# dmn-sjk/cones_perception

Hardware: NVIDIA B200
Metric: points/sec at 130k-pt scans (frames/sec and p50 frame latency in extra keys) (higher is better)
Workload: dtype f32

## Files before the change

### cones_perception_b200/csrc/frame_kernels.cuh

```cuda
#pragma once
#include "cluster_kernels.cuh"
#include "common.cuh"
#include "stream_kernels.cuh"
#include "voxel_kernels.cuh"

namespace cp {

constexpr int kFrameThreadsMax = 512;

#ifdef CP_PHASE_CLOCKS
#define CP_PHASE(name)                                                          \
  do {                                                                          \
    __syncthreads();                                                            \
    if (tid == 0 && f == 0 && clk_n < 16) {                                     \
      clk_name[clk_n] = name;                                                   \
      clk_t[clk_n++] = clock64();                                               \
    }                                                                           \
  } while (0)
#else
#define CP_PHASE(name) do { } while (0)
#endif

struct FrameArgs {
  u32 n_frames;
  const uint8_t* in;
  Layout layout;
  Geom geom;
  const u32* mask;
  const u32* rowmax;
  const u32* low_key;
  CropK crop;
  GroundK gk;
  u32* rows_loaded;
  const u32* c_off;
  u32* gcount;
  int pad_survives;
  VoxelK vk;
  ClusterK ck;
  VoxelFrame* vf;
  u32* v_off;
  u32* k_off;
  u32* ncomp_f;
  u32* kcount_f;
  u32* ncrop_f;
  ClusterRec* slots;
  ClusterRec* direct_out;
  u32 direct_cap;
  u32* nvox_f;
  u32* fc;
  int counted_ground;
  u64* desc_v;
  Ctl* ctl;
  u32* ticket;
  float4* tap_vox;
  u32 tap_vox_cap;
  u32* tap_keys;
  u32* tap_order;
  i32* tap_labels;
};

template <int CMAX, int VMAX, int T>
struct FrameSmem {
// ... 70 lines not shown
    total += t;
  }
  return woff + inc - v;
}

template <int CMAX, int VMAX, int MODE, int T>
__device__ __forceinline__ void frame_process(const FrameArgs& a, FrameSmem<CMAX, VMAX, T>& s, const u32 f) {
  constexpr int kFrameThreads = T;
  const u32 tid = threadIdx.x;
  const int lane = lane_id(), warp = tid >> 5;
  {
#ifdef CP_PHASE_CLOCKS
    const char* clk_name[16];
    long long clk_t[16];
    int clk_n = 0;
    const long long clk_0 = clock64();
#endif
    u32 tile0, ntiles, npts;
    u64 first;
    if (a.geom.uniform_n) {
      tile0 = f * a.geom.tpf;
      ntiles = a.geom.tpf;
      npts = a.geom.uniform_n;
      first = (u64)f * a.geom.uniform_n;
    } else {
      tile0 = a.geom.frame_tile0[f];
      ntiles = (f + 1 < a.n_frames ? a.geom.frame_tile0[f + 1] : a.geom.n_tiles) - tile0;
      npts = a.geom.frame_n[f];
      first = a.geom.frame_off[f];
    }
    const u32 c0 = a.c_off ? a.c_off[f] : 0u;

    if (tid < 8) s.bbox[tid] = tid < 4 ? 0xFFFFFFFFu : 0u;
    if (tid == 0) {
      s.slow = 0;
      s.gkept = 0;
    }
    const bool fused = a.mask == nullptr;
    const bool do_ground = fused && a.gk.do_ground != 0;
    if (warp == 0) {
      float t = 0.0f;
      if (do_ground && lane < kNSect) {
        t = __double2float_ru((double)ord2f(__ldcg(&a.low_key[f * kSectStride + lane])) + 0.1);
        s.thr[lane] = t;
      }
      float mn = (do_ground && lane < kNSect) ? t : __int_as_float(0x7f800000);
      float mx = (do_ground && lane < kNSect) ? t : -__int_as_float(0x7f800000);
#pragma unroll
      for (int o2 = 16; o2; o2 >>= 1) {
        mn = fminf(mn, __shfl_xor_sync(kFull, mn, o2));
        mx = fmaxf(mx, __shfl_xor_sync(kFull, mx, o2));
      }
      if (lane == 0) {
        s.thr[31] = do_ground ? mn : -__int_as_float(0x7f800000);
        s.thr[30] = do_ground ? mx : -__int_as_float(0x7f800000);
      }
    }
    __syncthreads();
    u32 C = 0;
    {
      constexpr u32 CH = 4u * CMAX;
      constexpr u32 RPT = CH / kFrameThreads;
      static_assert(CH % kFrameThreads == 0 && RPT % 8 == 0 && RPT <= 32, "chunk rows per thread");
      static_assert(sizeof(s.u) >= CH * sizeof(unsigned short), "live-row list must fit the scratch union");
      u32* mword = reinterpret_cast<u32*>(&s.px[0]);
      unsigned short* liverow = reinterpret_cast<unsigned short*>(&s.u);
      const u32 nrows = (npts + 31u) >> 5;
      const float thr_min = s.thr[31], thr_max = s.thr[30];
      const u32 key_min = f2ord(thr_min);
      const bool skipping = do_ground && a.rowmax != nullptr;
      u32 mnx = 0xFFFFFFFFu, mny = 0xFFFFFFFFu, mnz = 0xFFFFFFFFu, mxx = 0, mxy = 0, mxz = 0;
      u32 gkept = 0;
      for (u32 cb = 0; cb < nrows; cb += CH) {
        const u32 nr = nrows - cb < CH ? nrows - cb : CH;
        const u32 r0 = tid * RPT;
        u32 w[RPT];
        if (!fused) {
#pragma unroll
          for (u32 q = 0; q < RPT; q += 4) {
            uint4 m = make_uint4(0u, 0u, 0u, 0u);
            if (r0 + q < nr) m = *reinterpret_cast<const uint4*>(a.mask + (u64)tile0 * kTileWords + cb + r0 + q);
            w[q] = m.x; w[q + 1] = m.y; w[q + 2] = m.z; w[q + 3] = m.w;
          }
        } else {
          u32 live = 0;
#pragma unroll
          for (u32 q = 0; q < RPT; q += 4) {
            uint4 m = make_uint4(0xFFFFFFFFu, 0xFFFFFFFFu, 0xFFFFFFFFu, 0xFFFFFFFFu);
            if (skipping && r0 + q < nr)
              m = __ldcg(reinterpret_cast<const uint4*>(a.rowmax + (u64)tile0 * kTileWords + cb + r0 + q));
            live |= (m.x >= key_min ? 1u : 0u) << q;
            live |= (m.y >= key_min ? 1u : 0u) << (q + 1);
            live |= (m.z >= key_min ? 1u : 0u) << (q + 2);
            live |= (m.w >= key_min ? 1u : 0u) << (q + 3);
          }
          if (r0 + RPT > nr) live &= r0 < nr ? (0xFFFFFFFFu >> (32u - (nr - r0))) : 0u;
#pragma unroll
          for (u32 q = 0; q < RPT; ++q) mword[r0 + q] = 0u;
          u32 nlive;
          u32 lp = block_excl_scan<T>(__popc(live), s.wsum, nlive);
          while (live) {
            const u32 b = (u32)__ffs(live) - 1u;
            live &= live - 1;
            liverow[lp++] = (unsigned short)(r0 + b);
          }
          if (tid == 0) s.nlive = nlive;
          __syncthreads();
          CP_PHASE("live rows");
          constexpr u32 KB = T == 256 ? 4 : 8;
          for (u32 e0 = (u32)warp * KB; e0 < nlive; e0 += (kFrameThreads / 32) * KB) {
            float4 p[KB];
            u32 row[KB];
#pragma unroll
            for (u32 j = 0; j < KB; ++j) {
              row[j] = e0 + j < nlive ? (u32)liverow[e0 + j] : 0xFFFFFFFFu;
              const u32 i = (cb + row[j]) * 32u + lane;
              p[j] = (row[j] != 0xFFFFFFFFu && i < npts) ? load_point<MODE>(a.in, first + i, a.layout)
                                                          : make_float4(0.f, 0.f, -__int_as_float(0x7f800000), 0.f);
            }
#pragma unroll
            for (u32 j = 0; j < KB; ++j) {
              if (row[j] == 0xFFFFFFFFu) break;
              const u32 i = (cb + row[j]) * 32u + lane;
              const u32 bal = __ballot_sync(kFull, keep_point(p[j], i < npts, a.crop, a.gk, s.thr, thr_min, thr_max, gkept));
              if (lane == 0) mword[row[j]] = bal;
            }
          }
          __syncthreads();
          CP_PHASE("pass 2");
// ... 515 lines not shown
```

### cones_perception_b200/csrc/pipeline.cu

```cuda
#include "../../include/conesgpu.h"

#include <math.h>
#include <stdio.h>
#include <string.h>
#include <time.h>

#include <algorithm>
#include <memory>
#include <new>
#include <string>
#include <vector>

#include "cluster_front.cuh"
#include "cluster_kernels.cuh"
#include "color_kernels.cuh"
#include "color_net.cuh"
#include "common.cuh"
#include "copy_pool.hpp"
#include "frame_kernels.cuh"
#include "plane_kernels.cuh"
#include "radix_sort.cuh"
#include "single_frame.cuh"
#include "stream_kernels.cuh"
#include "tflite_reader.hpp"
// ... 130 lines not shown
  const uint8_t* in_ptr = nullptr;
  Layout layout{};
  const uint8_t* run_in = nullptr;
  Layout run_layout{};
  bool plane_on = false;
  cp_plane_params plane{};
  double plane_cos = 0.0;
  bool plane_run = false;
  bool plane_valid = false;
  u32 plane_frames = 0, plane_h = 0;
  PlaneBufs pb{};
  HostGeom hg;
  u32 *d_frame_n = nullptr, *d_frame_tile0 = nullptr, *d_tile_frame = nullptr;
  u64* d_frame_off = nullptr;
  u32 *d_low_key = nullptr, *d_bbox = nullptr, *d_c_off = nullptr, *d_gcount = nullptr, *d_v_off = nullptr;
  u32 *d_ncomp_f = nullptr, *d_kcount_f = nullptr, *d_k_off = nullptr;
  VoxelFrame* d_vf = nullptr;
  float4* d_pts = nullptr;
  u32 *d_src = nullptr, *d_frame = nullptr;
  u64 *d_keys_a = nullptr, *d_keys_b = nullptr, *d_okeys_a = nullptr, *d_okeys_b = nullptr;
  u32 *d_vals_a = nullptr, *d_vals_b = nullptr, *d_ovals_a = nullptr, *d_ovals_b = nullptr;
  u32 *d_sort_hdr = nullptr, *d_sort_state = nullptr;
  u32 *d_vstart = nullptr, *d_cstart = nullptr, *d_comp_start = nullptr;
  float4* d_vox = nullptr;
  u32 *d_vox_frame = nullptr, *d_parent = nullptr, *d_label = nullptr;
  u64* d_hkeys = nullptr;
  u32* d_hvals = nullptr;
  ClusterRec* d_clusters = nullptr;
  u32 *d_mask = nullptr, *d_tile_count = nullptr, *d_tile_excl = nullptr;
  float* d_thr_f = nullptr;
  u32* d_rowmax = nullptr;
  bool rowmax_valid = false;
  bool use_rowskip = true;
  bool use_single = true;
  bool self_published = false;
  bool graph_self_published = false;
  u64 hint_c = 0, hint_v = 0;
  cp_ground_params rp_ground{};
  bool rp_has_ground = false;
  bool tail_priority = false;
  int prio_low = 0;
  int k1_ctas_per_sm = 0;
  int frame_ctas_per_sm = 0;
  bool tile_ctas = true;
  u32 run_sgrid = 0;
  int stream_ctas_per_sm = 8;
  u64 *d_desc_a = nullptr, *d_desc_b = nullptr, *d_desc_c = nullptr, *d_desc_d = nullptr;
  u32 *d_tap_keys = nullptr, *d_tap_order = nullptr;
  i32* d_tap_labels = nullptr;
  uint8_t* h_stage[2] = {nullptr, nullptr};
  bool stage_streaming = true;
  int stage_threads = 1;
  std::unique_ptr<CopyPool> copy_pool;
  Ctl* h_ctl = nullptr;
  u32* h_frame_u32 = nullptr;
  std::vector<void*> dev_allocs, pin_allocs;
};

namespace {

#define CK(call)                                                                              \
  do {                                                                                        \
    cudaError_t e_ = (call);                                                                  \
    if (e_ != cudaSuccess) {                                                                  \
      char buf_[512];                                                                         \
      snprintf(buf_, sizeof(buf_), "%s:%d %s -> %s", __FILE__, __LINE__, #call,               \
               cudaGetErrorString(e_));                                                       \
      h->err = buf_;                                                                          \
      return CP_E_CUDA;                                                                       \
    }                                                                                         \
  } while (0)

template <typename T>
cp_status dalloc(cp_handle* h, T** p, size_t count) {
  void* q = nullptr;
// ... 106 lines not shown
  k->r2 = (float)((double)tol_f * (double)tol_f);
  if (!(tol_f > 0.0f) || !isfinite(tol_f)) {
    h->err = "cone_width/cone_height give a non-positive or non-finite cluster tolerance";
    return CP_E_PARAM;
  }
  const double edge = (double)tol_f * 0.505;
  double reach = fabs(d->distance_treshold_max);
  if (!(reach < 1e6)) {
    h->err = "distance_treshold_max must be finite and below 1e6 m";
    return CP_E_PARAM;
  }
  reach += 4 * edge;
  const u64 nx = (u64)ceil(2.0 * reach / edge) + 2;
  k->inv_h = (float)(1.0 / ((double)tol_f * 1.01));
  k->inv_g = (float)(1.0 / edge);
  k->origin = (float)reach;
  k->nx = (u32)nx;
  const u64 cells = (u64)n_frames * nx * nx * nx;
  if (nx > (1u << 20) || ceil_log2_host(cells) > 60) {
    h->err = "neighbour grid too large for 64-bit cell keys";
    return CP_E_PARAM;
  }
  *csort_bits = ceil_log2_host(cells);
  if (*csort_bits == 0) *csort_bits = 1;
  k->min_size = d->min_cluster_size < 0 ? 0u : (u32)d->min_cluster_size;
  k->max_size = d->max_cluster_size < 0 ? 0u : (u32)d->max_cluster_size;
  k->frame_bits = ceil_log2_host(n_frames);
  k->size_bits = ceil_log2_host((u64)k->max_size + 1);
  *osort_bits = k->frame_bits + k->size_bits + 1;
  return CP_OK;
}

__global__ void init_kernel(Ctl* ctl, u32 n_frames, float default_low, u32* low_key, u32* bbox, u32* c_off,
                            u32* gcount, u32* ncomp_f, u32* kcount_f, u64* desc_a, u32 na, u64* desc_b,
                            u64* desc_c, u64* desc_d, u32 nb) {
  const u32 t = blockIdx.x * blockDim.x + threadIdx.x, stride = gridDim.x * blockDim.x;
  if (t == 0) {
    Ctl z;
    memset(&z, 0, sizeof(z));
    *ctl = z;
    c_off[0] = 0;
  }
  const u32 lk = f2ord(default_low);
  for (u32 i = t; i < n_frames * kSectStride; i += stride) low_key[i] = lk;
  for (u32 i = t; i < n_frames * 8; i += stride) bbox[i] = ((i & 7u) < 4u) ? 0xFFFFFFFFu : 0u;
  for (u32 i = t; i < n_frames; i += stride) {
    gcount[i] = 0;
    ncomp_f[i] = 0;
    kcount_f[i] = 0;
    c_off[i + 1] = 0;
  }
  for (u32 i = t; i < na; i += stride) desc_a[i] = 0;
  for (u32 i = t; i < nb; i += stride) {
    desc_b[i] = 0;
    desc_c[i] = 0;
    desc_d[i] = 0;
  }
}

__global__ void tap_voxel_kernel(const Ctl* ctl, const u64* keys_a, const u64* keys_b, const u32* vals_a,
                                 const u32* vals_b, u32* tap_keys, u32* tap_order) {
  const u32 n = ctl->n_surv;
  const bool inb = sorted_in_b(ctl->vsort_bits);
  const u64* keys = inb ? keys_b : keys_a;
  const u32* vals = inb ? vals_b : vals_a;
  const u64 mask = (ctl->voxel_key_bits >= 64) ? ~0ull : ((1ull << ctl->voxel_key_bits) - 1ull);
  for (u32 i = blockIdx.x * blockDim.x + threadIdx.x; i < n; i += gridDim.x * blockDim.x) {
    tap_keys[i] = (u32)(keys[i] & mask);
    tap_order[i] = vals[i];
  }
}

cp_status check_view(cp_handle* h, const cp_cloud_view* v) {
  if (!v) {
    h->err = "NULL cloud view";
    return CP_E_PARAM;
  }
  const u64 n = (u64)v->width * v->height;
  if (n && !v->data) {
    h->err = "cloud view has points but a NULL data pointer";
// ... 97 lines not shown
  g.frame_off = h->d_frame_off;
  g.tile_frame = h->d_tile_frame;
  g.frame_tile0 = h->d_frame_tile0;
  return g;
}

u64 hinted(u64 cap, u64 hint) { return hint ? std::min<u64>(cap, 2 * hint + 8192) : cap; }

u32 grid_for(u64 work, u32 block, int sms, int per_sm) {
  u64 b = (work + block - 1) / block;
  if (b == 0) b = 1;
  const u64 cap = (u64)sms * per_sm;
  return (u32)(b < cap ? b : cap);
}

void launch_keep_mask(cp_handle* h, const Geom& g, const CropK& c, const GroundK& gk, u32 grid) {
  MaskOut mo;
  mo.mask = h->d_mask;
  mo.tile_count = h->d_tile_count;
  mo.gcount = h->d_gcount;
  mo.rows_loaded = &h->d_ctl->rows_loaded;
  if (gk.do_ground) {
    ground_thresholds_kernel<<<(g.n_frames + 127) / 128, 128, 0, h->stream>>>(g.n_frames, h->d_low_key, h->d_thr_f);
    h->launches++;
  }
  cudaMemsetAsync(h->d_mask, 0, sizeof(u32) * (size_t)g.n_tiles * kTileWords, h->stream);
  cudaMemsetAsync(h->d_tile_count, 0, sizeof(u32) * g.n_tiles, h->stream);
  if (h->stage_timing) cudaEventRecord(h->ev_k[2], h->stream);
  const u32 total_warps = (u32)h->sms * 4u * kStreamWarps;
  u32 split_log2 = 0;
  while (split_log2 < 3 && (((u64)g.n_tiles * 2u) << (split_log2 + 1)) <= total_warps) ++split_log2;
  if (split_log2) grid = grid_for((((u64)g.n_tiles * 2u) << split_log2) * 32u, kStreamThreads, h->sms, h->stream_ctas_per_sm);
  const u32* rm = h->rowmax_valid ? h->d_rowmax : nullptr;
  switch (h->run_layout.mode) {
    case 0: keep_mask_kernel<0><<<grid, kStreamThreads, 0, h->stream>>>(h->run_in, h->run_layout, g, c, gk, h->d_thr_f, rm, mo, split_log2); break;
    case 1: keep_mask_kernel<1><<<grid, kStreamThreads, 0, h->stream>>>(h->run_in, h->run_layout, g, c, gk, h->d_thr_f, rm, mo, split_log2); break;
    default: keep_mask_kernel<2><<<grid, kStreamThreads, 0, h->stream>>>(h->run_in, h->run_layout, g, c, gk, h->d_thr_f, rm, mo, split_log2); break;
  }
  if (h->stage_timing) cudaEventRecord(h->ev_k[3], h->stream);
  h->launches++;
  h->masked = true;
}

void launch_scan_gather(cp_handle* h, const Geom& g, const GroundK& gk, u32 cap) {
  GatherOut go;
  go.pts = h->d_pts;
  go.src = h->d_src;
  go.frame = h->d_frame;
  go.cap = cap;
  go.bbox_key = h->d_bbox;
  go.out32 = nullptr;
  const u32 stiles = (g.n_tiles + kScanTile - 1) / kScanTile;
  tile_scan_kernel<<<(h->tile_ctas || stiles < (u32)h->sms * 4) ? stiles : (u32)h->sms * 4, kScanThreads, 0, h->stream>>>(
      g, h->d_tile_count, h->d_tile_excl, h->d_c_off, h->d_desc_a, h->d_ctl, cap);
  const u32 ggrid = grid_for((u64)g.n_tiles * 32, 256, h->sms, 8);
  switch (h->run_layout.mode) {
    case 0: gather_survivors_kernel<0><<<ggrid, 256, 0, h->stream>>>(h->run_in, h->run_layout, g, gk, h->d_mask, h->d_tile_count, h->d_tile_excl, go); break;
    case 1: gather_survivors_kernel<1><<<ggrid, 256, 0, h->stream>>>(h->run_in, h->run_layout, g, gk, h->d_mask, h->d_tile_count, h->d_tile_excl, go); break;
    default: gather_survivors_kernel<2><<<ggrid, 256, 0, h->stream>>>(h->run_in, h->run_layout, g, gk, h->d_mask, h->d_tile_count, h->d_tile_excl, go); break;
  }
  h->launches += 2;
  h->gathered = true;
}
template <bool OUT32>
void launch_mask_compact(cp_handle* h, const Geom& g, const CropK& c, const GroundK& gk, u32 cap, uint8_t* out32) {
  GatherOut go;
  go.pts = h->d_pts;
  go.src = h->d_src;
  go.frame = h->d_frame;
  go.cap = cap;
  go.bbox_key = h->d_bbox;
// ... 83 lines not shown
void launch_front_fused(cp_handle* h, const Geom& g, const CropK& c, const GroundK& gk) {
  MaskOut mo;
  mo.mask = h->d_mask;
  mo.tile_count = h->d_tile_count;
  mo.gcount = h->d_gcount;
  mo.rows_loaded = &h->d_ctl->rows_loaded;
  if (h->fused_grid == 0) {
    int occ = 0;
    cudaOccupancyMaxActiveBlocksPerMultiprocessor(&occ, front_fused_kernel<0>, kStreamThreads, 0);
    if (occ < 1) occ = 1;
    h->fused_grid = (u32)(h->sms * occ);
  }
  FusedArgs fa;
  const u32 gf = (h->fused_grid + g.tpf - 1) / g.tpf;
  fa.group_tiles = gf * g.tpf;
  fa.n_groups = (g.n_frames + gf - 1) / gf;
  fa.done = h->d_done;
  fa.ticket = h->d_frame_ticket + 1;
  cudaMemsetAsync(h->d_done, 0, sizeof(u32) * g.n_frames, h->stream);
  cudaMemsetAsync(h->d_frame_ticket + 1, 0, sizeof(u32), h->stream);
  const u32 items = fa.n_groups * fa.group_tiles * 2u;
  const u32 grid = items < h->fused_grid ? items : h->fused_grid;
  if (h->stage_timing) cudaEventRecord(h->ev_k[0], h->stream);
  switch (h->run_layout.mode) {
    case 0: front_fused_kernel<0><<<grid, kStreamThreads, 0, h->stream>>>(h->run_in, h->run_layout, g, c, gk, h->d_low_key, mo, fa); break;
    case 1: front_fused_kernel<1><<<grid, kStreamThreads, 0, h->stream>>>(h->run_in, h->run_layout, g, c, gk, h->d_low_key, mo, fa); break;
    default: front_fused_kernel<2><<<grid, kStreamThreads, 0, h->stream>>>(h->run_in, h->run_layout, g, c, gk, h->d_low_key, mo, fa); break;
  }
  if (h->stage_timing) cudaEventRecord(h->ev_k[1], h->stream);
  h->launches++;
}

template <int MODE>
void launch_sector_min_mode(cp_handle* h, const Geom& g, u32 grid) {
  if (!h->tail_priority) {
    ground_sector_min_kernel<MODE><<<grid, kStreamThreads, 0, h->stream>>>(h->run_in, h->run_layout, g, h->d_low_key, h->d_rowmax);
    return;
  }
  cudaLaunchConfig_t cfg = {};
  cfg.gridDim = dim3(grid);
  cfg.blockDim = dim3(kStreamThreads);
  cfg.stream = h->stream;
  cudaLaunchAttribute at[1];
  at[0].id = cudaLaunchAttributePriority;
  at[0].val.priority = h->prio_low;
  cfg.attrs = at;
  cfg.numAttrs = 1;
  cudaLaunchKernelEx(&cfg, ground_sector_min_kernel<MODE>, h->run_in, h->run_layout, g, h->d_low_key, h->d_rowmax);
}
void launch_sector_min(cp_handle* h, const Geom& g, u32 grid) {
  if (h->k1_ctas_per_sm)
    grid = grid_for((u64)g.n_tiles * kStreamThreads, kStreamThreads, h->sms, h->k1_ctas_per_sm);
  switch (h->run_layout.mode) {
    case 0: launch_sector_min_mode<0>(h, g, grid); break;
    case 1: launch_sector_min_mode<1>(h, g, grid); break;
    default: launch_sector_min_mode<2>(h, g, grid); break;
  }
}

void launch_init(cp_handle* h, float default_low) {
  const u32 nb = (u32)(h->cap_c / kHeadTile + 2);
  init_kernel<<<h->sms * 2, 256, 0, h->stream>>>(h->d_ctl, h->hg.n_frames, default_low, h->d_low_key, h->d_bbox,
                                                 h->d_c_off, h->d_gcount, h->d_ncomp_f, h->d_kcount_f,
                                                 h->d_desc_a, h->hg.n_tiles, h->d_desc_b, h->d_desc_c, h->d_desc_d, nb);
  cudaMemsetAsync(h->d_desc_fv, 0, sizeof(u64) * h->hg.n_frames, h->stream);
  h->launches++;
}

SortArgs sort_args(cp_handle* h, bool order_sort, const u32* d_n, const u32* d_bits) {
  SortArgs a;
  a.keys_a = order_sort ? h->d_okeys_a : h->d_keys_a;
  a.keys_b = order_sort ? h->d_okeys_b : h->d_keys_b;
  a.vals_a = order_sort ? h->d_ovals_a : h->d_vals_a;
  a.vals_b = order_sort ? h->d_ovals_b : h->d_vals_b;
  a.d_n = d_n;
  a.d_bits = d_bits;
  a.hdr = h->d_sort_hdr;
  a.state = h->d_sort_state;
  a.tiles_cap = h->sort_tiles_cap;
  return a;
}

__global__ void back_reset_kernel(Ctl* ctl, u32 n_frames, u32* ncomp_f, u32* kcount_f) {
  const u32 t = blockIdx.x * blockDim.x + threadIdx.x;
  if (t == 0) {
    ctl->n_vox = ctl->n_cells = ctl->n_comp = ctl->n_clusters = 0;
    ctl->voxel_key_bits = 0;
    ctl->fast_overflow = 0;
    ctl->pairs_visited = ctl->pairs_tested = 0;
    ctl->error &= kErrSurvivors;
  }
  for (u32 i = t; i < n_frames; i += gridDim.x * blockDim.x) {
    ncomp_f[i] = 0;
    kcount_f[i] = 0;
  }
}
// ... 141 lines not shown

template <int CMAX, int VMAX, int MODE, int T>
void launch_frame_kernel(cp_handle* h, const FrameArgs& fa) {
  const size_t smem = sizeof(FrameSmem<CMAX, VMAX, T>);
  constexpr int kMaxDevices = 64;
  static int per_sm_dev[kMaxDevices] = {0};
  const int dev = (h->cfg.device >= 0 && h->cfg.device < kMaxDevices) ? h->cfg.device : 0;
  if (per_sm_dev[dev] == 0) {
    int per_sm = 1;
    cudaFuncSetAttribute(frame_backend_kernel<CMAX, VMAX, MODE, T>, cudaFuncAttributeMaxDynamicSharedMemorySize,
                         (int)smem);
    if (cudaOccupancyMaxActiveBlocksPerMultiprocessor(&per_sm, frame_backend_kernel<CMAX, VMAX, MODE, T>, T, smem) !=
            cudaSuccess || per_sm < 1)
      per_sm = 1;
    per_sm_dev[dev] = per_sm;
  }
  const int per_sm = h->frame_ctas_per_sm ? std::min(h->frame_ctas_per_sm, per_sm_dev[dev]) : per_sm_dev[dev];
  const u32 grid = std::min<u32>(fa.n_frames, (u32)h->sms * (u32)per_sm);
  if (h->stage_timing && !h->capturing) cudaEventRecord(h->ev_k[4], h->stream);
  frame_backend_kernel<CMAX, VMAX, MODE, T><<<grid, T, smem, h->stream>>>(fa);
  if (h->stage_timing && !h->capturing) cudaEventRecord(h->ev_k[5], h->stream);
  h->ran_frame_kernel = true;
  h->launches++;
}

FrameArgs frame_args(cp_handle* h, const RunParams& rp) {
  FrameArgs fa;
  fa.n_frames = h->hg.n_frames;
  fa.in = h->run_in;
  fa.layout = h->run_layout;
  fa.geom = device_geom(h);
  fa.mask = h->run_fused_mask ? nullptr : h->d_mask;
  fa.rowmax = h->rowmax_valid ? h->d_rowmax : nullptr;
  fa.low_key = h->d_low_key;
  fa.crop = rp.crop;
  fa.gk = rp.gk;
  fa.rows_loaded = &h->d_ctl->rows_loaded;
  fa.c_off = h->taps ? h->d_c_off : nullptr;
  fa.gcount = h->d_gcount;
  fa.pad_survives = rp.gk.pad_survives;
  fa.vk = rp.vk;
  fa.ck = rp.ck;
  fa.vf = h->d_vf;
  fa.v_off = h->d_v_off;
  fa.k_off = h->d_k_off;
  fa.ncomp_f = h->d_ncomp_f;
  fa.kcount_f = h->d_kcount_f;
  fa.ncrop_f = h->d_ncrop_f;
  fa.slots = h->d_slots;
  const bool direct = fa.n_frames == 1;
  fa.direct_out = direct ? reinterpret_cast<ClusterRec*>(h->d_clusters) : nullptr;
  fa.direct_cap = (u32)std::min<u64>(h->cap_v, 0xFFFFFFFFu);
  fa.fc = h->d_fc;
  fa.counted_ground = h->counted_ground ? 1 : 0;
  fa.nvox_f = h->d_nvox_f;
  fa.desc_v = h->d_desc_fv;
  fa.ctl = h->d_ctl;
  fa.ticket = h->d_frame_ticket;
  fa.tap_vox = h->taps ? h->d_vox : nullptr;
  fa.tap_vox_cap = (u32)h->cap_v;
  fa.tap_keys = h->taps ? h->d_tap_keys : nullptr;
  fa.tap_order = h->taps ? h->d_tap_order : nullptr;
  fa.tap_labels = h->taps ? h->d_tap_labels : nullptr;
  return fa;
}

// ... 14 lines not shown
  cfg.dynamicSmemBytes = kSfMaxPtsPerCta * 3 * sizeof(float);
  cfg.stream = h->stream;
  cfg.attrs = attr;
  cfg.numAttrs = 1;
  auto kern = single_frame_kernel<CMAX, VMAX, MODE>;
  if (!ready[dev]) {
    ready[dev] = true;
    const size_t max_smem = std::max<size_t>(cfg.dynamicSmemBytes, sizeof(FrameSmem<CMAX, VMAX, kSfThreads>));
    int n = 0;
    cfg.dynamicSmemBytes = max_smem;
    usable[dev] = cudaFuncSetAttribute(kern, cudaFuncAttributeMaxDynamicSharedMemorySize, (int)max_smem) == cudaSuccess &&
                  cudaFuncSetAttribute(kern, cudaFuncAttributeNonPortableClusterSizeAllowed, 1) == cudaSuccess &&
                  cudaOccupancyMaxActiveClusters(&n, kern, &cfg) == cudaSuccess && n >= 1;
    cudaGetLastError();
  }
  if (!usable[dev]) return false;
  cfg.dynamicSmemBytes = smem;
  if (cudaLaunchKernelEx(&cfg, kern, a) != cudaSuccess) {
    cudaGetLastError();
    return false;
  }
  return true;
}

bool single_frame_eligible(const cp_handle* h, const Geom& g) {
  return h->use_single && !h->plane_run && g.n_frames == 1 && g.uniform_n != 0 && h->run_layout.mode <= 1 && !h->taps && !h->stage_timing &&
         h->back_mode < 3 && !h->gather.open && g.uniform_n <= (u32)kSfCluster * kSfMaxPtsPerCta;
}

bool launch_single_frame(cp_handle* h, const RunParams& rp, float default_low) {
  SingleArgs a;
  h->run_fused_mask = false;
  h->rowmax_valid = false;
  a.fa = frame_args(h, rp);
  a.n = h->hg.uniform_n;
  const u32 per = (a.n + kSfCluster - 1) / kSfCluster;
  a.pts_per_cta = (per + kSfSub - 1) / kSfSub * kSfSub;
  a.default_low = default_low;
  a.o.mask = h->d_mask;
  a.o.tile_count = h->d_tile_count;
  a.o.gcount = h->d_gcount;
  a.o.rows_loaded = &h->d_ctl->rows_loaded;
  a.low_key = h->d_low_key;
  a.h_ctl = reinterpret_cast<u32*>(h->h_ctl);
  a.h_fc = h->h_fc;
  a.h_res = h->h_result;
  a.off_words = (u32)h->off_words;
  a.max_records = (u32)std::min<u64>(h->prefetch_cap, 0xFFFFFFFFu);
  const size_t stash = (size_t)a.pts_per_cta * 3 * sizeof(float);
  bool ok;
#define CP_SF(CM, VM)                                                                                         \
  do {                                                                                                        \
    const size_t smem = std::max(stash, sizeof(FrameSmem<CM, VM, kSfThreads>));                               \
    ok = h->run_layout.mode == 0 ? launch_single_frame_t<CM, VM, 0>(h, a, smem) : launch_single_frame_t<CM, VM, 1>(h, a, smem); \
  } while (0)
  if (h->back_mode == 0) CP_SF(1024, 512);
  else if (h->back_mode == 1) CP_SF(2048, 1024);
  else CP_SF(4096, 2048);
#undef CP_SF
  return ok;
}

template <int CMAX, int VMAX, int T>
void enqueue_back_fast(cp_handle* h, const RunParams& rp) {
  FrameArgs fa = frame_args(h, rp);
  const bool direct = fa.n_frames == 1;
// ... 207 lines not shown
  h->rp.d = *d;
  h->rp.vk = vk;
  h->rp.ck = ck;
  h->rp.gk = gk;
  h->rp.crop = crop;
  h->rp.csort_bits = csort_bits;
  h->rp.osort_bits = osort_bits;
  h->rp_has_ground = ground != nullptr;
  if (ground) h->rp_ground = *ground;
  h->self_published = false;
  if (single_frame_eligible(h, g)) {
    h->ran_cluster = h->ran_fused = false;
    if (launch_single_frame(h, h->rp, ground ? ground->default_lowest_point : 0.0f)) {
      h->masked = true;
      h->gathered = false;
      h->ran_ground = ground != nullptr;
      h->ran_frame_kernel = true;
      h->launches = 1;
      h->self_published = true;
      h->fetched = true;
      h->prefetched = h->prefetch_cap;
      h->ran = true;
      return CP_OK;
    }
  }
  if (!h->capturing) cudaEventRecord(h->ev0, h->stream);
  launch_init(h, ground ? ground->default_lowest_point : 0.0f);
  if (plane) {
    st = enqueue_plane_node(h, false);
    if (st) return st;
  }
  h->masked = false;
  h->run_fused_mask = false;
  h->ran_frame_kernel = false;
  const u32 sgrid = grid_for((u64)g.n_tiles * kStreamThreads, kStreamThreads, h->sms, h->stream_ctas_per_sm);
  h->run_sgrid = sgrid;
  h->ran_cluster = cluster_front_eligible(h, g, ground != nullptr) &&
                   launch_front_cluster(h, g, crop, gk, ground->default_lowest_point);
  h->ran_fused = !h->ran_cluster && ground && g.uniform_n && h->use_fused;
  if (h->ran_cluster) {
    h->masked = true;
  } else if (h->ran_fused) {
    launch_front_fused(h, g, crop, gk);
    h->masked = true;
  } else {
    h->rowmax_valid = false;
    if (ground) {
      if (h->stage_timing) cudaEventRecord(h->ev_k[0], h->stream);
      launch_sector_min(h, g, sgrid);
      if (h->stage_timing) cudaEventRecord(h->ev_k[1], h->stream);
      h->launches++;
      h->rowmax_valid = h->use_rowskip;
    }
    h->run_fused_mask = h->fuse_mask && h->back_mode < 3 &&
                        (ground != nullptr || plane || g.n_frames >= (u32)h->sms || h->fuse_mask_always);
    if (!h->run_fused_mask && h->back_mode < 3) launch_keep_mask(h, g, crop, gk, sgrid);
  }
  h->gathered = false;
  h->ran_ground = ground != nullptr;
  if (h->gather.open) h->gather.seq++;
  st = enqueue_back(h, false);
  if (st) return st;
  h->ran = true;
  return CP_OK;
}

constexpr size_t kParallelStageMin = 512ull << 10;
constexpr size_t kStagePiece = 64ull << 10;
cp_status stage_parallel(cp_handle* h, const uint8_t* src, size_t total, size_t dst_off, int* ring) {
  if (!h->copy_pool) {
    try {
      h->copy_pool.reset(new CopyPool(h->stage_threads - 1));
    } catch (...) {
      h->stage_threads = 1;
      return CP_E_STATE;
    }
  }
  size_t done = 0;
  while (done < total) {
    const size_t chunk = std::min(kStageChunk, total - done);
    const int r = *ring;
    CK(cudaEventSynchronize(h->ev_stage[r]));
// ... 465 lines not shown
  A(dalloc(h, &h->d_ovals_b, h->cap_v));
  A(dalloc(h, &h->d_sort_state, (size_t)2 * kRadix * h->sort_tiles_cap));
  A(dalloc(h, &h->d_sort_hdr, kSortHdrWords * 4));
  A(dalloc(h, &h->d_vstart, h->cap_v));
  A(dalloc(h, &h->d_cstart, h->cap_v));
  A(dalloc(h, &h->d_comp_start, h->cap_v));
  A(dalloc(h, &h->d_vox, h->cap_v));
  A(dalloc(h, &h->d_vox_frame, h->cap_v));
  A(dalloc(h, &h->d_parent, h->cap_v));
  A(dalloc(h, &h->d_label, h->cap_v));
  A(dalloc(h, &h->d_hkeys, h->hash_cap));
  A(dalloc(h, &h->d_hvals, h->hash_cap));
  {
    const size_t off_words = ((size_t)F + 1 + 3) / 4 * 4;
    u32* block = nullptr;
    A(dalloc(h, &block, off_words + (size_t)h->cap_v * 4));
    h->d_k_off = block;
    h->d_clusters = reinterpret_cast<ClusterRec*>(block + off_words);
    h->off_words = off_words;
    h->prefetch_cap = std::min<u64>(h->cap_v, 1ull << 20);
    A(palloc(h, &h->h_result, off_words + 4 * (size_t)h->prefetch_cap));
    A(dalloc(h, &h->d_fc, (size_t)F * 8));
    A(palloc(h, &h->h_fc, (size_t)F * 8));
  }
  A(dalloc(h, &h->d_desc_a, h->tiles_cap));
  A(dalloc(h, &h->d_frame_ticket, 2));
  A(dalloc(h, &h->d_done, F));
  A(dalloc(h, &h->d_ncrop_f, F));
  A(dalloc(h, &h->d_nvox_f, F));
  A(dalloc(h, &h->d_slots, (size_t)F * 2048));
  A(dalloc(h, &h->d_desc_fv, F));
  A(dalloc(h, &h->d_mask, (size_t)h->tiles_cap * kTileWords));
  A(dalloc(h, &h->d_rowmax, (size_t)h->tiles_cap * kTileWords));
  A(dalloc(h, &h->d_thr_f, (size_t)F * kSectStride));
  A(dalloc(h, &h->d_tile_count, h->tiles_cap));
  A(dalloc(h, &h->d_tile_excl, h->tiles_cap));
  const size_t nb = h->cap_c / kHeadTile + 2;
  A(dalloc(h, &h->d_desc_b, nb));
  A(dalloc(h, &h->d_desc_c, nb));
  A(dalloc(h, &h->d_desc_d, nb));
  if (h->taps) {
    A(dalloc(h, &h->d_tap_keys, h->cap_c));
    A(dalloc(h, &h->d_tap_order, h->cap_c));
    A(dalloc(h, &h->d_tap_labels, h->cap_v));
  }
  A(palloc(h, &h->h_stage[0], kStageChunk));
  A(palloc(h, &h->h_stage[1], kStageChunk));
  A(palloc(h, &h->h_ctl, 1));
  A(palloc(h, &h->h_frame_u32, std::max<size_t>((size_t)(F + 1) * 8, (size_t)kSectStride)));
#undef A
  memset(h->h_ctl, 0, sizeof(Ctl));
  *out = h;
  return CP_OK;
} catch (...) {
  return abi_exception(nullptr);
}

void cp_destroy(cp_handle* h) {
  if (!h) return;
  cudaSetDevice(h->cfg.device);
  if (h->stream) cudaStreamSynchronize(h->stream);
  if (h->gather.open && !h->gather.owner && h->gather.base) cudaIpcCloseMemHandle(h->gather.base);
  for (void* p : h->dev_allocs) cudaFree(p);
  for (void* p : h->pin_allocs) cudaFreeHost(p);
  if (h->d_out32) cudaFree(h->d_out32);
  for (void* q : {(void*)h->color.mask, (void*)h->color.tcount, (void*)h->color.texcl, (void*)h->color.off,
// ... 342 lines not shown
  st = cp_batch_run(h, d, ground);
  if (st) return st;
  return cp_batch_results(h, counters, cluster_offsets, out, cap, n_total);
} catch (...) {
  return abi_exception(h);
}

cp_status cp_detect(cp_handle* h, const cp_cloud_view* in, const cp_detect_params* d, const cp_ground_params* ground,
                    cp_cluster* out, uint32_t cap, uint32_t* n_clusters, cp_frame_counters* counters) try {
  if (!h) return CP_E_PARAM;
  if (!n_clusters) {
    h->err = "NULL n_clusters";
    return CP_E_PARAM;
  }
  uint64_t total = 0;
  cp_status st = cp_detect_batch(h, in, 1, d, ground, counters, nullptr, out, cap, &total);
  *n_clusters = (uint32_t)total;
  return st;
} catch (...) {
  return abi_exception(h);
}

namespace {
cp_status enqueue_ground(cp_handle* h, const cp_ground_params* g) {
  cp_status st = ensure_out32(h);
  if (st) return st;
  const Geom geo = device_geom(h);
  h->launches = 0;
  h->key_valid = false;
  h->plane_run = false;
  h->run_in = h->in_ptr;
  h->run_layout = h->layout;
  launch_init(h, g->default_lowest_point);
  if (h->plane_on) return enqueue_plane_node(h, true);
  h->plane_valid = false;
  const u32 sgrid = grid_for((u64)geo.n_tiles * kStreamThreads, kStreamThreads, h->sms, 8);
  launch_sector_min(h, geo, sgrid);
  h->launches++;
  h->rowmax_valid = h->use_rowskip;
  CropK crop;
  memset(&crop, 0, sizeof(crop));
  GroundK gk;
  gk.do_ground = 1;
  gk.want_count = 1;
  gk.pad_survives = 0;
  launch_mask_compact<true>(h, geo, crop, gk, (u32)h->hg.n_points, h->d_out32);
  return CP_OK;
}

void fill_pad_host(cp_handle* h, uint8_t* out8, size_t out_bytes) {
  if (h->stage_threads > 1 && out_bytes >= kParallelStageMin) {
    if (!h->copy_pool) {
      try {
        h->copy_pool.reset(new CopyPool(h->stage_threads - 1));
      } catch (...) {
        h->stage_threads = 1;
      }
    }
    if (h->copy_pool) {
      std::shared_ptr<CopyPool::Batch> b = h->copy_pool->start(out8, nullptr, out_bytes, kStagePiece, 1, true);
      b->work();
      for (u32 gi = 0; gi < b->n_groups; ++gi)
        while (!b->group_done(gi)) std::this_thread::yield();
      return;
    }
  }
  fill_pad_points(out8, out_bytes);
}
}

// ... 1151 lines not shown
```

### cones_perception_b200/csrc/stream_kernels.cuh

```cuda
#pragma once
#include "common.cuh"

namespace cp {

constexpr int kStreamThreads = 256;
constexpr int kStreamWarps = kStreamThreads / 32;
constexpr int kStreamRows = 8;
constexpr int kStreamTile = kStreamThreads * kStreamRows;
constexpr int kTileWords = kStreamTile / 32;

struct Layout {
  u32 step;
  i32 ox, oy, oz, oi;
  u32 mode;
};

struct Geom {
  u32 n_frames;
  u32 uniform_n;
  u32 tpf;
  u32 n_tiles;
  const u32* frame_n;
  const u64* frame_off;
  const u32* tile_frame;
// ... 220 lines not shown
  }
  __syncthreads();
}

template <int MODE>
__device__ __forceinline__ void load_tile(const uint8_t* __restrict__ in, const Layout& L, u64 base, u32 count,
                                          float pad_z, float4 (&p)[kStreamRows], u32 rows = 0xFFu) {
  const u32 wbase = (threadIdx.x >> 5) * (32 * kStreamRows) + lane_id();
#pragma unroll
  for (int r = 0; r < kStreamRows; ++r) {
    const u32 i = wbase + r * 32;
    p[r] = ((i < count) && ((rows >> r) & 1u)) ? load_point<MODE>(in, base + i, L)
                                                : make_float4(0.f, 0.f, pad_z, 0.f);
  }
}

__device__ __forceinline__ void sector_min_tile(const float4 (&p)[kStreamRows], u32* smin, const u32* s_bound) {
#pragma unroll
  for (int r = 0; r < kStreamRows; ++r) {
    const u32 zk = f2ord(p[r].z);
    const float x = p[r].x, y = p[r].y;
    const u32 q = (x * y == 0.0f) ? 0u : 1u + (x < 0.0f ? 1u : 0u) + (y < 0.0f ? 2u : 0u);
    if (zk < s_bound[q]) {
      if (finite3(x, y, p[r].z)) {
        bool ok;
        const float a = atan2_approx(y, x, ok);
        const int s = sector_of(x, y, a, ok);
        if (zk < smin[s]) atomicMin(&smin[s], zk);
      }
    }
  }
}

template <int MODE>
__global__ void __launch_bounds__(kStreamThreads, 4)
ground_sector_min_kernel(const uint8_t* __restrict__ in, Layout L, Geom g, u32* __restrict__ low_key,
                         u32* __restrict__ rowmax) {
  __shared__ u32 smin[kSectStride];
  const u32 per = (g.n_tiles + gridDim.x - 1) / gridDim.x;
  const u32 t0 = blockIdx.x * per;
  const u32 t1 = t0 + per < g.n_tiles ? t0 + per : g.n_tiles;
  const int lane = lane_id();
  u32 cur_frame = 0xFFFFFFFFu;
  for (u32 tile = t0; tile < t1; ++tile) {
    u32 frame, local0, count;
    u64 first;
    tile_lookup(g, tile, frame, local0, count, first);
    if (frame != cur_frame) {
      __syncthreads();
      if (cur_frame != 0xFFFFFFFFu && threadIdx.x < kNSect)
        atomicMin(&low_key[cur_frame * kSectStride + threadIdx.x], smin[threadIdx.x]);
      if (threadIdx.x < kSectStride)
        smin[threadIdx.x] = threadIdx.x < kNSect ? __ldcg(&low_key[frame * kSectStride + threadIdx.x]) : 0u;
      cur_frame = frame;
      __syncthreads();
    }
    float4 p[kStreamRows];
    load_tile<MODE>(in, L, first + local0, count, __int_as_float(0x7f800000), p);
    const u32 v = lane < kNSect ? *(volatile const u32*)&smin[lane] : 0u;
    const u32 ball = __reduce_max_sync(kFull, v);
    const u32 b1 = __reduce_max_sync(kFull, lane <= 4 ? v : 0u);
    const u32 b2 = __reduce_max_sync(kFull, (lane >= 4 && lane <= 8) ? v : 0u);
    const u32 b3 = __reduce_max_sync(kFull, (lane >= 12 && lane <= 16) ? v : 0u);
    const u32 b4 = __reduce_max_sync(kFull, (lane >= 8 && lane <= 12) ? v : 0u);
    u32 mine = 0;
#pragma unroll
    for (int r = 0; r < kStreamRows; ++r) {
      const u32 zk = f2ord(p[r].z);
      if (__reduce_min_sync(kFull, zk) < ball) {
        const float x = p[r].x, y = p[r].y;
        const u32 bq = (x * y == 0.0f) ? ball : (y < 0.0f ? (x < 0.0f ? b4 : b3) : (x < 0.0f ? b2 : b1));
        if (zk < bq && finite3(x, y, p[r].z)) {
          bool ok;
          const float a = atan2_approx(y, x, ok);
          const int s = sector_of(x, y, a, ok);
          if (zk < smin[s]) atomicMin(&smin[s], zk);
        }
      }
      const u32 m = __reduce_max_sync(kFull, zk);
      if (lane == r) mine = m;
    }
    if (rowmax && lane < kStreamRows) rowmax[(u64)tile * kTileWords + (threadIdx.x >> 5) * kStreamRows + lane] = mine;
  }
  __syncthreads();
  if (cur_frame != 0xFFFFFFFFu && threadIdx.x < kNSect)
    atomicMin(&low_key[cur_frame * kSectStride + threadIdx.x], smin[threadIdx.x]);
}

__device__ __forceinline__ bool crop_keep(const CropK& c, float x, float y, float z) {
  if (z < c.zthr) return false;
  const float sf = fmaf(z, z, fmaf(y, y, x * x));
  bool exact = !(sf < 1e30f);
  exact |= (sf > c.smax_lo) & (sf < c.smax_hi);
  exact |= (sf > c.smin_lo) & (sf < c.smin_hi);
  if (exact) {
    const double xd = x, yd = y, zd = z;
    double s = __dadd_rn(__dmul_rn(xd, xd), __dmul_rn(yd, yd));
    s = __dadd_rn(s, __dmul_rn(zd, zd));
    return !(s >= c.smax || s < c.smin);
  }
  return !(sf >= c.smax_hi || sf <= c.smin_lo);
}

struct MaskOut {
  u32* mask;
  u32* tile_count;
  u32* gcount;
  u32* rows_loaded;
};

__device__ __forceinline__ void ground_thresholds(const u32* __restrict__ low_key, u32 frame, float* thr,
                                                  float* thr_min) {
  const int lane = lane_id();
  if ((threadIdx.x >> 5) == 0) {
    float t = __int_as_float(0x7f800000);
    if (lane < kNSect) {
      t = __double2float_ru((double)ord2f(__ldcg(&low_key[frame * kSectStride + lane])) + 0.1);
      thr[lane] = t;
    }
// ... 85 lines not shown
    if (gkeep) {
      gkept++;
      keep = !c.do_crop || crop_keep(c, x, y, z);
      if (keep && c.do_crop) {
        if (!have_a) a = atan2_approx(y, x, ok);
        const float aa = fabsf(a);
        if (!ok | (aa > c.f_lo_guard)) {
          if (ok & (aa >= c.f_hi_guard)) keep = false;
          else keep = fabsf(atan2_exact(y, x)) < c.f_hi;
        }
      }
    }
  }
  return keep;
}

__global__ void ground_thresholds_kernel(u32 n_frames, const u32* __restrict__ low_key, float* __restrict__ thr_f) {
  const u32 f = blockIdx.x * blockDim.x + threadIdx.x;
  if (f >= n_frames) return;
  float mn = __int_as_float(0x7f800000), mx = -__int_as_float(0x7f800000);
  for (int s = 0; s < kNSect; ++s) {
    const float t = __double2float_ru((double)ord2f(low_key[f * kSectStride + s]) + 0.1);
    thr_f[f * kSectStride + s] = t;
    mn = fminf(mn, t);
    mx = fmaxf(mx, t);
  }
  thr_f[f * kSectStride + 31] = mn;
  thr_f[f * kSectStride + 30] = mx;
}

template <int MODE>
__global__ void __launch_bounds__(kStreamThreads, 4)
keep_mask_kernel(const uint8_t* __restrict__ in, Layout L, Geom g, CropK c, GroundK gk,
                 const float* __restrict__ thr_f, const u32* __restrict__ rowmax, MaskOut o, u32 split_log2) {
  constexpr int kBatch = 4;
  const int lane = lane_id();
  const u32 nwarps = gridDim.x * kStreamWarps;
  const u32 gw = blockIdx.x * kStreamWarps + (threadIdx.x >> 5);
  const u32 ngroups = g.n_tiles * 2u;
  const bool skipping = gk.do_ground && rowmax != nullptr;
  u32 nrows = 0;
  const u32 nvg = ngroups << split_log2;
  const u32 slice_rows = 32u >> split_log2;
  for (u32 round = 0, g0 = 0; g0 < nvg; ++round, g0 += nwarps) {
    const u32 vg = g0 + (gw + round * 37u) % nwarps;
    if (vg >= nvg) continue;
    const u32 grp = vg >> split_log2, sub = vg & ((1u << split_log2) - 1u);
    const u32 slice = split_log2 ? (((1u << slice_rows) - 1u) << (sub * slice_rows)) : 0xFFFFFFFFu;
    const u32 rk = skipping ? rowmax[(u64)grp * 32 + lane] : 0xFFFFFFFFu;
    const u32 tile = grp >> 1;
    u32 frame, local0, count;
    u64 first;
    tile_lookup(g, tile, frame, local0, count, first);
    const float* thr = thr_f + (size_t)frame * kSectStride;
    const float thr_min = gk.do_ground ? __ldg(thr + 31) : -__int_as_float(0x7f800000);
    const float thr_max = gk.do_ground ? __ldg(thr + 30) : -__int_as_float(0x7f800000);
    const u32 half0 = (grp & 1u) * (kStreamTile / 2);
    if (gk.pad_survives && (grp & 1u) && lane == 0 && sub == 0 &&
        (local0 + count) == (g.uniform_n ? g.uniform_n : g.frame_n[frame]))
      atomicAdd(&o.tile_count[tile], 1u);
    u32 todo = __ballot_sync(kFull, rk >= f2ord(thr_min)) & slice;
    if (todo == 0) continue;
    nrows += __popc(todo);
    const u32 live = todo;
    u32 myword = 0, gcount = 0, gkept = 0;
    if (todo == 0xFFFFFFFFu) {
#pragma unroll 1
      for (u32 b = 0; b < 4; ++b) {
        float4 p[kStreamRows];
#pragma unroll
        for (int r = 0; r < kStreamRows; ++r) {
          const u32 i = half0 + (b * kStreamRows + r) * 32 + lane;
          p[r] = (i < count) ? load_point<MODE>(in, first + local0 + i, L)
                             : make_float4(0.f, 0.f, -__int_as_float(0x7f800000), 0.f);
        }
#pragma unroll
        for (int r = 0; r < kStreamRows; ++r) {
          const u32 i = half0 + (b * kStreamRows + r) * 32 + lane;
          const u32 bal = __ballot_sync(kFull, keep_point(p[r], i < count, c, gk, thr, thr_min, thr_max, gkept));
          gcount += __popc(bal);
          if ((u32)lane == b * kStreamRows + r) myword = bal;
        }
      }
      todo = 0;
    }
    while (todo) {
      float4 p[kBatch];
      u32 rowid[kBatch];
#pragma unroll
      for (int j = 0; j < kBatch; ++j) {
        rowid[j] = todo ? (u32)__ffs(todo) - 1u : 0xFFFFFFFFu;
        todo &= todo - 1;
        const u32 i = half0 + rowid[j] * 32 + lane;
        p[j] = (rowid[j] != 0xFFFFFFFFu && i < count) ? load_point<MODE>(in, first + local0 + i, L)
// ... 440 lines not shown
```

Baseline: 320.4 billion.

## Mark rows settled in sector-min pass and skip them in mask/frame kernels

During the ground sector-min pass, each warp row whose points all lie above the ground ceiling and beyond the crop's maximum radius is flagged as settled, and the count of such points is accumulated per frame. The keep-mask and frame kernels then drop settled rows from their live sets and add the precomputed count to the ground-kept tally, so they never reload or re-test those points. This adds a per-row byte array, extra per-frame atomics and a bitmask load per row group. It also sets the default k1 CTAs per SM to 3.

```diff
diff --git a/cones_perception_b200/csrc/frame_kernels.cuh b/cones_perception_b200/csrc/frame_kernels.cuh
--- a/cones_perception_b200/csrc/frame_kernels.cuh
+++ b/cones_perception_b200/csrc/frame_kernels.cuh
@@ -28,6 +28,8 @@
   Geom geom;
   const u32* mask;
   const u32* rowmax;
+  const uint8_t* settled;
+  const u32* settled_kept;
   const u32* low_key;
   CropK crop;
   GroundK gk;
@@ -164,11 +166,11 @@
     const u32 c0 = a.c_off ? a.c_off[f] : 0u;
 
     if (tid < 8) s.bbox[tid] = tid < 4 ? 0xFFFFFFFFu : 0u;
+    const bool fused = a.mask == nullptr;
     if (tid == 0) {
       s.slow = 0;
-      s.gkept = 0;
-    }
-    const bool fused = a.mask == nullptr;
+      s.gkept = (fused && a.settled) ? __ldcg(&a.settled_kept[f]) : 0u;
+    }
     const bool do_ground = fused && a.gk.do_ground != 0;
     if (warp == 0) {
       float t = 0.0f;
@@ -227,6 +229,12 @@
             live |= (m.w >= key_min ? 1u : 0u) << (q + 3);
           }
           if (r0 + RPT > nr) live &= r0 < nr ? (0xFFFFFFFFu >> (32u - (nr - r0))) : 0u;
+          if (a.settled && r0 < nr) {
+            const uint8_t* sb = a.settled + (((u64)tile0 * kTileWords + cb + r0) >> 3);
+            const u32 sv = RPT == 32 ? __ldcg(reinterpret_cast<const unsigned int*>(sb))
+                         : RPT == 16 ? (u32)__ldcg(reinterpret_cast<const unsigned short*>(sb)) : (u32)__ldcg(sb);
+            live &= ~sv;
+          }
 #pragma unroll
           for (u32 q = 0; q < RPT; ++q) mword[r0 + q] = 0u;
           u32 nlive;
diff --git a/cones_perception_b200/csrc/pipeline.cu b/cones_perception_b200/csrc/pipeline.cu
--- a/cones_perception_b200/csrc/pipeline.cu
+++ b/cones_perception_b200/csrc/pipeline.cu
@@ -186,6 +186,9 @@
   u32* d_rowmax = nullptr;
   bool rowmax_valid = false;
   bool use_rowskip = true;
+  uint8_t* d_settled = nullptr;
+  u32* d_settled_kept = nullptr;
+  bool settle_valid = false;
   bool use_single = true;
   bool self_published = false;
   bool graph_self_published = false;
@@ -194,7 +197,7 @@
   bool rp_has_ground = false;
   bool tail_priority = false;
   int prio_low = 0;
-  int k1_ctas_per_sm = 0;
+  int k1_ctas_per_sm = 3;
   int frame_ctas_per_sm = 0;
   bool tile_ctas = true;
   u32 run_sgrid = 0;
@@ -367,7 +370,7 @@
 }
 
 __global__ void init_kernel(Ctl* ctl, u32 n_frames, float default_low, u32* low_key, u32* bbox, u32* c_off,
-                            u32* gcount, u32* ncomp_f, u32* kcount_f, u64* desc_a, u32 na, u64* desc_b,
+                            u32* gcount, u32* settled_kept, u32* ncomp_f, u32* kcount_f, u64* desc_a, u32 na, u64* desc_b,
                             u64* desc_c, u64* desc_d, u32 nb) {
   const u32 t = blockIdx.x * blockDim.x + threadIdx.x, stride = gridDim.x * blockDim.x;
   if (t == 0) {
@@ -381,6 +384,7 @@
   for (u32 i = t; i < n_frames * 8; i += stride) bbox[i] = ((i & 7u) < 4u) ? 0xFFFFFFFFu : 0u;
   for (u32 i = t; i < n_frames; i += stride) {
     gcount[i] = 0;
+    settled_kept[i] = 0;
     ncomp_f[i] = 0;
     kcount_f[i] = 0;
     c_off[i + 1] = 0;
@@ -544,11 +548,15 @@
   while (split_log2 < 3 && (((u64)g.n_tiles * 2u) << (split_log2 + 1)) <= total_warps) ++split_log2;
   if (split_log2) grid = grid_for((((u64)g.n_tiles * 2u) << split_log2) * 32u, kStreamThreads, h->sms, h->stream_ctas_per_sm);
   const u32* rm = h->rowmax_valid ? h->d_rowmax : nullptr;
+  const uint8_t* sr = h->settle_valid ? h->d_settled : nullptr;
+#define CP_KM(M) keep_mask_kernel<M><<<grid, kStreamThreads, 0, h->stream>>>(h->run_in, h->run_layout, g, c, gk, h->d_thr_f, \
+                                                                       rm, sr, h->d_settled_kept, mo, split_log2)
   switch (h->run_layout.mode) {
-    case 0: keep_mask_kernel<0><<<grid, kStreamThreads, 0, h->stream>>>(h->run_in, h->run_layout, g, c, gk, h->d_thr_f, rm, mo, split_log2); break;
-    case 1: keep_mask_kernel<1><<<grid, kStreamThreads, 0, h->stream>>>(h->run_in, h->run_layout, g, c, gk, h->d_thr_f, rm, mo, split_log2); break;
-    default: keep_mask_kernel<2><<<grid, kStreamThreads, 0, h->stream>>>(h->run_in, h->run_layout, g, c, gk, h->d_thr_f, rm, mo, split_log2); break;
-  }
+    case 0: CP_KM(0); break;
+    case 1: CP_KM(1); break;
+    default: CP_KM(2); break;
+  }
+#undef CP_KM
   if (h->stage_timing) cudaEventRecord(h->ev_k[3], h->stream);
   h->launches++;
   h->masked = true;
@@ -698,9 +706,10 @@
 }
 
 template <int MODE>
-void launch_sector_min_mode(cp_handle* h, const Geom& g, u32 grid) {
+void launch_sector_min_mode(cp_handle* h, const Geom& g, u32 grid, const Settle& st) {
   if (!h->tail_priority) {
-    ground_sector_min_kernel<MODE><<<grid, kStreamThreads, 0, h->stream>>>(h->run_in, h->run_layout, g, h->d_low_key, h->d_rowmax);
+    ground_sector_min_kernel<MODE><<<grid, kStreamThreads, 0, h->stream>>>(h->run_in, h->run_layout, g, h->d_low_key,
+                                                                           h->d_rowmax, st);
     return;
   }
   cudaLaunchConfig_t cfg = {};
@@ -712,22 +721,32 @@
   at[0].val.priority = h->prio_low;
   cfg.attrs = at;
   cfg.numAttrs = 1;
-  cudaLaunchKernelEx(&cfg, ground_sector_min_kernel<MODE>, h->run_in, h->run_layout, g, h->d_low_key, h->d_rowmax);
-}
-void launch_sector_min(cp_handle* h, const Geom& g, u32 grid) {
+  cudaLaunchKernelEx(&cfg, ground_sector_min_kernel<MODE>, h->run_in, h->run_layout, g, h->d_low_key, h->d_rowmax, st);
+}
+void launch_sector_min(cp_handle* h, const Geom& g, u32 grid, float default_low, const CropK* settle) {
   if (h->k1_ctas_per_sm)
     grid = grid_for((u64)g.n_tiles * kStreamThreads, kStreamThreads, h->sms, h->k1_ctas_per_sm);
+  Settle st;
+  memset(&st, 0, sizeof(st));
+  const float ceil = round_up_to_float((double)default_low + 0.1);
+  if (settle && settle->do_crop && std::isfinite(ceil) && std::isfinite(settle->smax)) {
+    st.ceil_key = f2ord(ceil);
+    st.smax_hi = settle->smax_hi;
+    st.settled = h->d_settled;
+    st.settled_kept = h->d_settled_kept;
+  }
+  h->settle_valid = st.settled != nullptr;
   switch (h->run_layout.mode) {
-    case 0: launch_sector_min_mode<0>(h, g, grid); break;
-    case 1: launch_sector_min_mode<1>(h, g, grid); break;
-    default: launch_sector_min_mode<2>(h, g, grid); break;
+    case 0: launch_sector_min_mode<0>(h, g, grid, st); break;
+    case 1: launch_sector_min_mode<1>(h, g, grid, st); break;
+    default: launch_sector_min_mode<2>(h, g, grid, st); break;
   }
 }
 
 void launch_init(cp_handle* h, float default_low) {
   const u32 nb = (u32)(h->cap_c / kHeadTile + 2);
   init_kernel<<<h->sms * 2, 256, 0, h->stream>>>(h->d_ctl, h->hg.n_frames, default_low, h->d_low_key, h->d_bbox,
-                                                 h->d_c_off, h->d_gcount, h->d_ncomp_f, h->d_kcount_f,
+                                                 h->d_c_off, h->d_gcount, h->d_settled_kept, h->d_ncomp_f, h->d_kcount_f,
                                                  h->d_desc_a, h->hg.n_tiles, h->d_desc_b, h->d_desc_c, h->d_desc_d, nb);
   cudaMemsetAsync(h->d_desc_fv, 0, sizeof(u64) * h->hg.n_frames, h->stream);
   h->launches++;
@@ -935,6 +954,8 @@
   fa.geom = device_geom(h);
   fa.mask = h->run_fused_mask ? nullptr : h->d_mask;
   fa.rowmax = h->rowmax_valid ? h->d_rowmax : nullptr;
+  fa.settled = h->settle_valid ? h->d_settled : nullptr;
+  fa.settled_kept = h->d_settled_kept;
   fa.low_key = h->d_low_key;
   fa.crop = rp.crop;
   fa.gk = rp.gk;
@@ -1015,6 +1036,7 @@
   SingleArgs a;
   h->run_fused_mask = false;
   h->rowmax_valid = false;
+  h->settle_valid = false;
   a.fa = frame_args(h, rp);
   a.n = h->hg.uniform_n;
   const u32 per = (a.n + kSfCluster - 1) / kSfCluster;
@@ -1288,6 +1310,7 @@
   }
   h->masked = false;
   h->run_fused_mask = false;
+  h->settle_valid = false;
   h->ran_frame_kernel = false;
   const u32 sgrid = grid_for((u64)g.n_tiles * kStreamThreads, kStreamThreads, h->sms, h->stream_ctas_per_sm);
   h->run_sgrid = sgrid;
@@ -1302,8 +1325,9 @@
   } else {
     h->rowmax_valid = false;
     if (ground) {
+      const bool settle = h->use_rowskip && h->back_mode < 3;
       if (h->stage_timing) cudaEventRecord(h->ev_k[0], h->stream);
-      launch_sector_min(h, g, sgrid);
+      launch_sector_min(h, g, sgrid, ground->default_lowest_point, settle ? &crop : nullptr);
       if (h->stage_timing) cudaEventRecord(h->ev_k[1], h->stream);
       h->launches++;
       h->rowmax_valid = h->use_rowskip;
@@ -1835,6 +1859,8 @@
   A(dalloc(h, &h->d_desc_fv, F));
   A(dalloc(h, &h->d_mask, (size_t)h->tiles_cap * kTileWords));
   A(dalloc(h, &h->d_rowmax, (size_t)h->tiles_cap * kTileWords));
+  A(dalloc(h, &h->d_settled, (size_t)h->tiles_cap * kStreamWarps));
+  A(dalloc(h, &h->d_settled_kept, F));
   A(dalloc(h, &h->d_thr_f, (size_t)F * kSectStride));
   A(dalloc(h, &h->d_tile_count, h->tiles_cap));
   A(dalloc(h, &h->d_tile_excl, h->tiles_cap));
@@ -2243,10 +2269,11 @@
   h->run_in = h->in_ptr;
   h->run_layout = h->layout;
   launch_init(h, g->default_lowest_point);
+  h->settle_valid = false;
   if (h->plane_on) return enqueue_plane_node(h, true);
   h->plane_valid = false;
   const u32 sgrid = grid_for((u64)geo.n_tiles * kStreamThreads, kStreamThreads, h->sms, 8);
-  launch_sector_min(h, geo, sgrid);
+  launch_sector_min(h, geo, sgrid, g->default_lowest_point, nullptr);
   h->launches++;
   h->rowmax_valid = h->use_rowskip;
   CropK crop;
diff --git a/cones_perception_b200/csrc/stream_kernels.cuh b/cones_perception_b200/csrc/stream_kernels.cuh
--- a/cones_perception_b200/csrc/stream_kernels.cuh
+++ b/cones_perception_b200/csrc/stream_kernels.cuh
@@ -276,11 +276,19 @@
   }
 }
 
+struct Settle {
+  u32 ceil_key;
+  float smax_hi;
+  uint8_t* settled;
+  u32* settled_kept;
+};
+
 template <int MODE>
 __global__ void __launch_bounds__(kStreamThreads, 4)
 ground_sector_min_kernel(const uint8_t* __restrict__ in, Layout L, Geom g, u32* __restrict__ low_key,
-                         u32* __restrict__ rowmax) {
+                         u32* __restrict__ rowmax, Settle st) {
   __shared__ u32 smin[kSectStride];
+  __shared__ u32 s_settled;
   const u32 per = (g.n_tiles + gridDim.x - 1) / gridDim.x;
   const u32 t0 = blockIdx.x * per;
   const u32 t1 = t0 + per < g.n_tiles ? t0 + per : g.n_tiles;
@@ -294,6 +302,10 @@
       __syncthreads();
       if (cur_frame != 0xFFFFFFFFu && threadIdx.x < kNSect)
         atomicMin(&low_key[cur_frame * kSectStride + threadIdx.x], smin[threadIdx.x]);
+      if (threadIdx.x == kNSect) {
+        if (cur_frame != 0xFFFFFFFFu && s_settled) atomicAdd(&st.settled_kept[cur_frame], s_settled);
+        s_settled = 0;
+      }
       if (threadIdx.x < kSectStride)
         smin[threadIdx.x] = threadIdx.x < kNSect ? __ldcg(&low_key[frame * kSectStride + threadIdx.x]) : 0u;
       cur_frame = frame;
@@ -307,11 +319,12 @@
     const u32 b2 = __reduce_max_sync(kFull, (lane >= 4 && lane <= 8) ? v : 0u);
     const u32 b3 = __reduce_max_sync(kFull, (lane >= 12 && lane <= 16) ? v : 0u);
     const u32 b4 = __reduce_max_sync(kFull, (lane >= 8 && lane <= 12) ? v : 0u);
-    u32 mine = 0;
+    u32 mine = 0, sbits = 0;
 #pragma unroll
     for (int r = 0; r < kStreamRows; ++r) {
       const u32 zk = f2ord(p[r].z);
-      if (__reduce_min_sync(kFull, zk) < ball) {
+      const u32 zmin = __reduce_min_sync(kFull, zk);
+      if (zmin < ball) {
         const float x = p[r].x, y = p[r].y;
         const u32 bq = (x * y == 0.0f) ? ball : (y < 0.0f ? (x < 0.0f ? b4 : b3) : (x < 0.0f ? b2 : b1));
         if (zk < bq && finite3(x, y, p[r].z)) {
@@ -320,15 +333,26 @@
           const int s = sector_of(x, y, a, ok);
           if (zk < smin[s]) atomicMin(&smin[s], zk);
         }
+      } else if (st.settled && zmin >= st.ceil_key) {
+        const float x = p[r].x, y = p[r].y, z = p[r].z;
+        const bool far = ((threadIdx.x >> 5) * (32 * kStreamRows) + r * 32 + lane < count) && finite3(x, y, z) &&
+                         fmaf(z, z, fmaf(y, y, x * x)) >= st.smax_hi;
+        if (__all_sync(kFull, far)) sbits |= 1u << r;
       }
       const u32 m = __reduce_max_sync(kFull, zk);
       if (lane == r) mine = m;
     }
     if (rowmax && lane < kStreamRows) rowmax[(u64)tile * kTileWords + (threadIdx.x >> 5) * kStreamRows + lane] = mine;
+    if (st.settled && lane == 0) {
+      st.settled[(u64)tile * kStreamWarps + (threadIdx.x >> 5)] = (uint8_t)sbits;
+      if (sbits) atomicAdd(&s_settled, 32u * (u32)__popc(sbits));
+    }
   }
   __syncthreads();
   if (cur_frame != 0xFFFFFFFFu && threadIdx.x < kNSect)
     atomicMin(&low_key[cur_frame * kSectStride + threadIdx.x], smin[threadIdx.x]);
+  if (cur_frame != 0xFFFFFFFFu && threadIdx.x == kNSect && s_settled)
+    atomicAdd(&st.settled_kept[cur_frame], s_settled);
 }
 
 __device__ __forceinline__ bool crop_keep(const CropK& c, float x, float y, float z) {
@@ -480,7 +504,8 @@
 template <int MODE>
 __global__ void __launch_bounds__(kStreamThreads, 4)
 keep_mask_kernel(const uint8_t* __restrict__ in, Layout L, Geom g, CropK c, GroundK gk,
-                 const float* __restrict__ thr_f, const u32* __restrict__ rowmax, MaskOut o, u32 split_log2) {
+                 const float* __restrict__ thr_f, const u32* __restrict__ rowmax, const uint8_t* __restrict__ settled,
+                 const u32* __restrict__ settled_kept, MaskOut o, u32 split_log2) {
   constexpr int kBatch = 4;
   const int lane = lane_id();
   const u32 nwarps = gridDim.x * kStreamWarps;
@@ -508,6 +533,13 @@
         (local0 + count) == (g.uniform_n ? g.uniform_n : g.frame_n[frame]))
       atomicAdd(&o.tile_count[tile], 1u);
     u32 todo = __ballot_sync(kFull, rk >= f2ord(thr_min)) & slice;
+    if (settled) {
+      todo &= ~__ldcg(reinterpret_cast<const u32*>(settled) + grp);
+      if (local0 == 0 && grp == tile * 2u && sub == 0 && lane == 0) {
+        const u32 sk = __ldcg(&settled_kept[frame]);
+        if (sk) atomicAdd(&o.gcount[frame], sk);
+      }
+    }
     if (todo == 0) continue;
     nrows += __popc(todo);
     const u32 live = todo;
```

Result: faster. 351.7 billion (median of 6 runs) (+9.8%).
